# francois-rozet/sda

Measured on AMD Instinct MI355X. Metric: diffusion-steps/s (Kolmogorov 64x256x256 posterior sampling; unit = one predictor-corrector step of a 16-trajectory per-GPU shard), higher is better.
Workload: dtype f32; 1 GPU; kolmogorov256; per_gpu_batch=16, global_batch=16, guided=True, corrections=1, schedule_steps=1000, hipgraph_step=True, observation=fused Subsample (hand-written adjoint; no autograd through A), corrector_noise=row-keyed Philox (sda_randn_rows), parallelism=dp1 (batch-sharded, no in-loop collective), ranks_seen=1, process_group_live=False

## Files before the change

### sda_amd/csrc/conv_few.hip

```cpp
#include "sda_common.hpp"
#include <stdlib.h>

#define CF_CK 16
#define CF_TR 8
#define CF_TW 32
#define CF_HR (CF_TR + 2)
#define CF_HC (CF_TW + 2)
#define CF_PLANE 368
#define CF_ROW 36
#define CF_NPOS (CF_HR * CF_HC)
#define CF_BUF (CF_CK * CF_PLANE + 9 * CF_CK * 16)

typedef float cf_f32x4 __attribute__((ext_vector_type(4)));
typedef float cf_f32x2 __attribute__((ext_vector_type(2)));

__global__ __launch_bounds__(512, 4) void conv_few_kernel(const sda_conv_desc d, int tiles_x, int tiles_y) {
    __shared__ __attribute__((aligned(16))) float smem[2 * CF_BUF];
    const int tid = threadIdx.x, lane = tid & 63, kq = lane >> 4, li = lane & 15;
    const int wave = __builtin_amdgcn_readfirstlane(tid >> 6);
    int t;
    {
        const int total = (int)gridDim.x, xcd = (int)blockIdx.x & 7, slot = (int)blockIdx.x >> 3;
        const int tq = total >> 3, tr = total & 7;
        t = xcd * tq + (xcd < tr ? xcd : tr) + slot;
    }
    const int bx = t % tiles_x; t /= tiles_x;
    const int by = t % tiles_y;
    const int n = t / tiles_y;
    const int oy0 = by * CF_TR, ox0 = bx * CF_TW;
    const int nstage = d.cin_pad / CF_CK;
    if (wave >= 4) {
        const int ptid = tid - 256;
        const int ng = n + d.x_n_off;
        const float* ximg = d.x + (int64_t)(ng / d.n_inner) * d.x_sn_outer + (int64_t)(ng % d.n_inner) * d.x_sn_inner;
        unsigned goff[2];
        int loff[2];
        bool live[2];
#pragma unroll
        for (int j = 0; j < 2; ++j) {
            const int pos = ptid + 256 * j;
            const bool valid = pos < CF_NPOS;
            const int hy = pos / CF_HC, hx = pos - hy * CF_HC;
            int y = oy0 - 1 + hy, x = ox0 - 1 + hx;
            bool ok = valid;
            if (d.circular) {
                y = y < 0 ? y + d.hs : (y >= d.hs ? y - d.hs : y);
                x = x < 0 ? x + d.ws : (x >= d.ws ? x - d.ws : x);
            } else {
                ok = ok && y >= 0 && y < d.hs && x >= 0 && x < d.ws;
            }
            goff[j] = (unsigned)((ok ? y : 0) * (int)d.x_sy + (ok ? x : 0) * (int)d.x_sx);
            loff[j] = valid ? hy * CF_ROW + hx : -1;
            live[j] = ok;
        }
        const int wch = ptid >> 4, wco = ptid & 15;
        const unsigned woff = (unsigned)(wch * d.cout_pad + wco);
        const int wdst = CF_CK * CF_PLANE + ((wch & 3) * 16 + wco) * 4 + (wch >> 2);
        const int64_t wtap = (int64_t)d.cin_pad * d.cout_pad;
        auto produce = [&](int st, float* buf) {
            const float* xs = ximg + (int64_t)(st * CF_CK) * d.x_sc;
            const float* ws = d.w + (int64_t)(st * CF_CK) * d.cout_pad;
            float vin[CF_CK][2], vw[9];
#pragma unroll
            for (int ch = 0; ch < CF_CK; ++ch) {
                vin[ch][0] = (xs + (int64_t)ch * d.x_sc)[goff[0]];
                vin[ch][1] = loff[1] >= 0 ? (xs + (int64_t)ch * d.x_sc)[goff[1]] : 0.f;
            }
#pragma unroll
            for (int tap = 0; tap < 9; ++tap) vw[tap] = (ws + tap * wtap)[woff];
            if (d.circular) {
#pragma unroll
                for (int ch = 0; ch < CF_CK; ++ch) {
                    buf[ch * CF_PLANE + loff[0]] = vin[ch][0];
                    if (loff[1] >= 0) buf[ch * CF_PLANE + loff[1]] = vin[ch][1];
                }
            } else {
#pragma unroll
                for (int ch = 0; ch < CF_CK; ++ch) {
                    buf[ch * CF_PLANE + loff[0]] = live[0] ? vin[ch][0] : 0.f;
                    if (loff[1] >= 0) buf[ch * CF_PLANE + loff[1]] = live[1] ? vin[ch][1] : 0.f;
                }
            }
#pragma unroll
            for (int tap = 0; tap < 9; ++tap) buf[wdst + tap * 256] = vw[tap];
        };
        produce(0, smem);
        __syncthreads();
        for (int st = 0; st < nstage; ++st) {
            if (st + 1 < nstage) produce(st + 1, smem + ((st + 1) & 1) * CF_BUF);
            __syncthreads();
        }
        return;
    }
    cf_f32x4 acc[4];
#pragma unroll
    for (int f = 0; f < 4; ++f) acc[f] = cf_f32x4{0.f, 0.f, 0.f, 0.f};
    const int brow = (2 * wave) * CF_ROW + li + kq * CF_PLANE;
    __syncthreads();
    for (int st = 0; st < nstage; ++st) {
        const float* buf = smem + (st & 1) * CF_BUF;
        const float* wl = buf + CF_CK * CF_PLANE + (kq * 16 + li) * 4;
#pragma unroll
        for (int half = 0; half < 2; ++half) {
            cf_f32x2 a[9];
#pragma unroll
            for (int tap = 0; tap < 9; ++tap) a[tap] = *reinterpret_cast<const cf_f32x2*>(wl + tap * 256 + 2 * half);
            float bb[2][4][6];
#pragma unroll
            for (int k2 = 0; k2 < 2; ++k2)
#pragma unroll
                for (int r = 0; r < 4; ++r)
#pragma unroll
                    for (int c = 0; c < 6; ++c)
                        bb[k2][r][c] = buf[brow + 4 * (2 * half + k2) * CF_PLANE + r * CF_ROW + 16 * (c / 3) + (c % 3)];
#pragma unroll
            for (int tap = 0; tap < 9; ++tap) {
                const int dy = tap / 3, dx = tap - 3 * dy;
#pragma unroll
                for (int k2 = 0; k2 < 2; ++k2)
#pragma unroll
                    for (int f = 0; f < 4; ++f)
                        acc[f] = __builtin_amdgcn_mfma_f32_16x16x4f32(a[tap][k2], bb[k2][(f >> 1) + dy][3 * (f & 1) + dx], acc[f], 0, 0, 0);
            }
        }
        __syncthreads();
    }
    const int64_t hw = (int64_t)d.ho * d.wo;
    float* on = d.out + (int64_t)n * d.cout * hw;
    const float* rn = d.res ? d.res + (int64_t)n * d.cout * hw : nullptr;
#pragma unroll
    for (int r = 0; r < 4; ++r) {
        const int co = 4 * kq + r;
        if (co >= d.cout) continue;
        const float bias = d.bias ? d.bias[co] : 0.f;
#pragma unroll
        for (int f = 0; f < 4; ++f) {
            const int64_t o = (int64_t)co * hw + (int64_t)(oy0 + 2 * wave + (f >> 1)) * d.wo + ox0 + 16 * (f & 1) + li;
            float v = acc[f][r] + bias;
            if (rn) v += rn[o];
            on[o] = v;
        }
    }
}

static bool few_ok(const sda_conv_desc* d) {
    static const bool off = getenv("SDA_CONV_FEW") && atoi(getenv("SDA_CONV_FEW")) == 0;
    if (off || !d || !d->x || !d->w || !d->out) return false;
    if (d->kh != 3 || d->kw != 3 || d->stride_h != 1 || d->stride_w != 1 || d->up_h != 1 || d->up_w != 1 || d->zins_h != 1 ||
        d->zins_w != 1 || d->explicit_pad || d->out_sn || d->out_sc || d->out_sy || d->out_sx)
        return false;
    if (d->cout < 1 || d->cout > 16 || d->cout_pad < 16 || d->cctx != 0 || d->mod || d->ln_mean || d->ln_rstd || d->act_in != SDA_ACT_NONE ||
        d->dact_z)
        return false;
    if (d->cin_pad % CF_CK || d->cx != d->cin_pad || d->n_inner < 1) return false;
    if (d->ho != d->hs || d->wo != d->ws || (d->ho % CF_TR) || (d->wo % CF_TW)) return false;
    if (d->x_sc < 0 || d->x_sy < 0 || d->x_sx < 0 ||
        (int64_t)d->cx * d->x_sc + (int64_t)d->hs * d->x_sy + (int64_t)d->ws * d->x_sx >= (1LL << 31))
        return false;
    if ((int64_t)9 * d->cin_pad * d->cout_pad >= (1LL << 31)) return false;
    const int64_t tiles = (int64_t)d->n * (d->ho / CF_TR) * (d->wo / CF_TW);
    return tiles >= 1 && tiles <= 0x7fffffffLL;
}

int sda_few_path(const sda_conv_desc* d) { return few_ok(d) ? 1 : 0; }

int sda_few_try(const sda_conv_desc* d, hipStream_t stream) {
    if (!few_ok(d)) return SDA_E_UNSUPPORTED;
    const int tx = d->wo / CF_TW, ty = d->ho / CF_TR;
    hipLaunchKernelGGL(conv_few_kernel, dim3((unsigned)((int64_t)d->n * tx * ty)), dim3(512), 0, stream, *d, tx, ty);
    return sda_launch_status();
}
```

Measured before the change: 0.1295 diffusion-steps/s.

## Make few-output conv kernel persistent with cross-tile producer prefetch

Caps the grid at two workgroups per CU and has each workgroup loop over several tiles in its XCD-local range. The producer waves prefetch the first channel stage of the next tile while the consumer waves finish the current one, so the pipeline does not drain between tiles, and per-workgroup setup such as bias loads happens once. This trades launch-level parallelism for lower fill and drain cost. Tile-to-XCD assignment and occupancy balance change, and per-workgroup serial work grows when there are few tiles.

```diff
diff --git a/sda_amd/csrc/conv_few.hip b/sda_amd/csrc/conv_few.hip
--- a/sda_amd/csrc/conv_few.hip
+++ b/sda_amd/csrc/conv_few.hip
@@ -10,49 +10,68 @@
 #define CF_ROW 36
 #define CF_NPOS (CF_HR * CF_HC)
 #define CF_BUF (CF_CK * CF_PLANE + 9 * CF_CK * 16)
+#define CF_WG_PER_CU 2
 
 typedef float cf_f32x4 __attribute__((ext_vector_type(4)));
 typedef float cf_f32x2 __attribute__((ext_vector_type(2)));
 
-__global__ __launch_bounds__(512, 4) void conv_few_kernel(const sda_conv_desc d, int tiles_x, int tiles_y) {
+struct cf_tile {
+    int bx, by, n;
+    __device__ __forceinline__ void set(int t, int tiles_x, int tiles_y) {
+        bx = t % tiles_x; t /= tiles_x;
+        by = t % tiles_y;
+        n = t / tiles_y;
+    }
+};
+
+__global__ __launch_bounds__(512, 4) void conv_few_kernel(const sda_conv_desc d, int tiles_x, int tiles_y, int tiles) {
     __shared__ __attribute__((aligned(16))) float smem[2 * CF_BUF];
     const int tid = threadIdx.x, lane = tid & 63, kq = lane >> 4, li = lane & 15;
     const int wave = __builtin_amdgcn_readfirstlane(tid >> 6);
-    int t;
+    int t0, ntile, tstep;
     {
         const int total = (int)gridDim.x, xcd = (int)blockIdx.x & 7, slot = (int)blockIdx.x >> 3;
-        const int tq = total >> 3, tr = total & 7;
-        t = xcd * tq + (xcd < tr ? xcd : tr) + slot;
-    }
-    const int bx = t % tiles_x; t /= tiles_x;
-    const int by = t % tiles_y;
-    const int n = t / tiles_y;
-    const int oy0 = by * CF_TR, ox0 = bx * CF_TW;
+        const int wgs = (total >> 3) + (xcd < (total & 7) ? 1 : 0);
+        const int tq = tiles >> 3, tr = tiles & 7;
+        const int x0 = xcd * tq + (xcd < tr ? xcd : tr), nx = tq + (xcd < tr ? 1 : 0);
+        t0 = x0 + slot;
+        tstep = wgs;
+        ntile = (nx - slot + wgs - 1) / wgs;
+    }
+    if (ntile <= 0) return;
+    cf_tile tl;
+    tl.set(t0, tiles_x, tiles_y);
     const int nstage = d.cin_pad / CF_CK;
     if (wave >= 4) {
         const int ptid = tid - 256;
-        const int ng = n + d.x_n_off;
-        const float* ximg = d.x + (int64_t)(ng / d.n_inner) * d.x_sn_outer + (int64_t)(ng % d.n_inner) * d.x_sn_inner;
+        int hy[2], hx[2];
+        int loff[2];
         unsigned goff[2];
-        int loff[2];
         bool live[2];
+        const float* ximg;
 #pragma unroll
         for (int j = 0; j < 2; ++j) {
             const int pos = ptid + 256 * j;
-            const bool valid = pos < CF_NPOS;
-            const int hy = pos / CF_HC, hx = pos - hy * CF_HC;
-            int y = oy0 - 1 + hy, x = ox0 - 1 + hx;
-            bool ok = valid;
-            if (d.circular) {
-                y = y < 0 ? y + d.hs : (y >= d.hs ? y - d.hs : y);
-                x = x < 0 ? x + d.ws : (x >= d.ws ? x - d.ws : x);
-            } else {
-                ok = ok && y >= 0 && y < d.hs && x >= 0 && x < d.ws;
-            }
-            goff[j] = (unsigned)((ok ? y : 0) * (int)d.x_sy + (ok ? x : 0) * (int)d.x_sx);
-            loff[j] = valid ? hy * CF_ROW + hx : -1;
-            live[j] = ok;
-        }
+            hy[j] = pos / CF_HC, hx[j] = pos - hy[j] * CF_HC;
+            loff[j] = pos < CF_NPOS ? hy[j] * CF_ROW + hx[j] : -1;
+        }
+        auto plan = [&]() {
+            const int ng = tl.n + d.x_n_off;
+            ximg = d.x + (int64_t)(ng / d.n_inner) * d.x_sn_outer + (int64_t)(ng % d.n_inner) * d.x_sn_inner;
+#pragma unroll
+            for (int j = 0; j < 2; ++j) {
+                int y = tl.by * CF_TR - 1 + hy[j], x = tl.bx * CF_TW - 1 + hx[j];
+                bool ok = loff[j] >= 0;
+                if (d.circular) {
+                    y = y < 0 ? y + d.hs : (y >= d.hs ? y - d.hs : y);
+                    x = x < 0 ? x + d.ws : (x >= d.ws ? x - d.ws : x);
+                } else {
+                    ok = ok && y >= 0 && y < d.hs && x >= 0 && x < d.ws;
+                }
+                goff[j] = (unsigned)((ok ? y : 0) * (int)d.x_sy + (ok ? x : 0) * (int)d.x_sx);
+                live[j] = ok;
+            }
+        };
         const int wch = ptid >> 4, wco = ptid & 15;
         const unsigned woff = (unsigned)(wch * d.cout_pad + wco);
         const int wdst = CF_CK * CF_PLANE + ((wch & 3) * 16 + wco) * 4 + (wch >> 2);
@@ -84,11 +103,22 @@
 #pragma unroll
             for (int tap = 0; tap < 9; ++tap) buf[wdst + tap * 256] = vw[tap];
         };
+        plan();
         produce(0, smem);
         __syncthreads();
-        for (int st = 0; st < nstage; ++st) {
-            if (st + 1 < nstage) produce(st + 1, smem + ((st + 1) & 1) * CF_BUF);
-            __syncthreads();
+        int par = 0;
+        for (int i = 0; i < ntile; ++i) {
+            for (int st = 0; st < nstage; ++st) {
+                par ^= 1;
+                if (st + 1 < nstage) {
+                    produce(st + 1, smem + par * CF_BUF);
+                } else if (i + 1 < ntile) {
+                    tl.set(t0 += tstep, tiles_x, tiles_y);
+                    plan();
+                    produce(0, smem + par * CF_BUF);
+                }
+                __syncthreads();
+            }
         }
         return;
     }
@@ -96,50 +126,59 @@
 #pragma unroll
     for (int f = 0; f < 4; ++f) acc[f] = cf_f32x4{0.f, 0.f, 0.f, 0.f};
     const int brow = (2 * wave) * CF_ROW + li + kq * CF_PLANE;
+    const int64_t hw = (int64_t)d.ho * d.wo;
+    float bias[4];
+#pragma unroll
+    for (int r = 0; r < 4; ++r) bias[r] = d.bias && 4 * kq + r < d.cout ? d.bias[4 * kq + r] : 0.f;
     __syncthreads();
-    for (int st = 0; st < nstage; ++st) {
-        const float* buf = smem + (st & 1) * CF_BUF;
-        const float* wl = buf + CF_CK * CF_PLANE + (kq * 16 + li) * 4;
-#pragma unroll
-        for (int half = 0; half < 2; ++half) {
-            cf_f32x2 a[9];
-#pragma unroll
-            for (int tap = 0; tap < 9; ++tap) a[tap] = *reinterpret_cast<const cf_f32x2*>(wl + tap * 256 + 2 * half);
-            float bb[2][4][6];
-#pragma unroll
-            for (int k2 = 0; k2 < 2; ++k2)
-#pragma unroll
-                for (int r = 0; r < 4; ++r)
-#pragma unroll
-                    for (int c = 0; c < 6; ++c)
-                        bb[k2][r][c] = buf[brow + 4 * (2 * half + k2) * CF_PLANE + r * CF_ROW + 16 * (c / 3) + (c % 3)];
-#pragma unroll
-            for (int tap = 0; tap < 9; ++tap) {
-                const int dy = tap / 3, dx = tap - 3 * dy;
+    int par = 0;
+    for (int i = 0; i < ntile; ++i) {
+        for (int st = 0; st < nstage; ++st) {
+            const float* buf = smem + par * CF_BUF;
+            const float* wl = buf + CF_CK * CF_PLANE + (kq * 16 + li) * 4;
+#pragma unroll
+            for (int half = 0; half < 2; ++half) {
+                cf_f32x2 a[9];
+#pragma unroll
+                for (int tap = 0; tap < 9; ++tap) a[tap] = *reinterpret_cast<const cf_f32x2*>(wl + tap * 256 + 2 * half);
+                float bb[2][4][6];
 #pragma unroll
                 for (int k2 = 0; k2 < 2; ++k2)
 #pragma unroll
-                    for (int f = 0; f < 4; ++f)
-                        acc[f] = __builtin_amdgcn_mfma_f32_16x16x4f32(a[tap][k2], bb[k2][(f >> 1) + dy][3 * (f & 1) + dx], acc[f], 0, 0, 0);
-            }
-        }
-        __syncthreads();
-    }
-    const int64_t hw = (int64_t)d.ho * d.wo;
-    float* on = d.out + (int64_t)n * d.cout * hw;
-    const float* rn = d.res ? d.res + (int64_t)n * d.cout * hw : nullptr;
-#pragma unroll
-    for (int r = 0; r < 4; ++r) {
-        const int co = 4 * kq + r;
-        if (co >= d.cout) continue;
-        const float bias = d.bias ? d.bias[co] : 0.f;
-#pragma unroll
-        for (int f = 0; f < 4; ++f) {
-            const int64_t o = (int64_t)co * hw + (int64_t)(oy0 + 2 * wave + (f >> 1)) * d.wo + ox0 + 16 * (f & 1) + li;
-            float v = acc[f][r] + bias;
-            if (rn) v += rn[o];
-            on[o] = v;
-        }
+                    for (int r = 0; r < 4; ++r)
+#pragma unroll
+                        for (int c = 0; c < 6; ++c)
+                            bb[k2][r][c] = buf[brow + 4 * (2 * half + k2) * CF_PLANE + r * CF_ROW + 16 * (c / 3) + (c % 3)];
+#pragma unroll
+                for (int tap = 0; tap < 9; ++tap) {
+                    const int dy = tap / 3, dx = tap - 3 * dy;
+#pragma unroll
+                    for (int k2 = 0; k2 < 2; ++k2)
+#pragma unroll
+                        for (int f = 0; f < 4; ++f)
+                            acc[f] = __builtin_amdgcn_mfma_f32_16x16x4f32(a[tap][k2], bb[k2][(f >> 1) + dy][3 * (f & 1) + dx], acc[f], 0, 0, 0);
+                }
+            }
+            __syncthreads();
+            par ^= 1;
+        }
+        float* on = d.out + (int64_t)tl.n * d.cout * hw;
+        const float* rn = d.res ? d.res + (int64_t)tl.n * d.cout * hw : nullptr;
+#pragma unroll
+        for (int r = 0; r < 4; ++r) {
+            const int co = 4 * kq + r;
+            if (co >= d.cout) continue;
+#pragma unroll
+            for (int f = 0; f < 4; ++f) {
+                const int64_t o = (int64_t)co * hw + (int64_t)(tl.by * CF_TR + 2 * wave + (f >> 1)) * d.wo + tl.bx * CF_TW + 16 * (f & 1) + li;
+                float v = acc[f][r] + bias[r];
+                if (rn) v += rn[o];
+                on[o] = v;
+            }
+        }
+#pragma unroll
+        for (int f = 0; f < 4; ++f) acc[f] = cf_f32x4{0.f, 0.f, 0.f, 0.f};
+        if (i + 1 < ntile) tl.set(t0 += tstep, tiles_x, tiles_y);
     }
 }
 
@@ -167,6 +206,10 @@
 int sda_few_try(const sda_conv_desc* d, hipStream_t stream) {
     if (!few_ok(d)) return SDA_E_UNSUPPORTED;
     const int tx = d->wo / CF_TW, ty = d->ho / CF_TR;
-    hipLaunchKernelGGL(conv_few_kernel, dim3((unsigned)((int64_t)d->n * tx * ty)), dim3(512), 0, stream, *d, tx, ty);
+    const int64_t tiles = (int64_t)d->n * tx * ty;
+    const int cus = sda_cu_count();
+    if (cus <= 0) return SDA_E_BADARG;
+    const int64_t resident = (int64_t)cus * CF_WG_PER_CU;
+    hipLaunchKernelGGL(conv_few_kernel, dim3((unsigned)(tiles < resident ? tiles : resident)), dim3(512), 0, stream, *d, tx, ty, (int)tiles);
     return sda_launch_status();
 }
```

After: 0.1297 diffusion-steps/s, median of 2. No clear change (+0.2%).
